# payakorn/InteriorPointMethod

Hardware: AMD Instinct MI355X
Metric: IPM iterations/sec (m=4096,n=8192 dense LP) (higher is better)
Workload: dtype f64; 1 GPU; dense synthetic LP m=4096 n=8192 fp64, seed 0, start x=s=1 y=0 (BASELINE.json configs[1]); replicas per GPU

## Files before the change

interiorpointmethod_amd/csrc/ff_schedule.h:

```cpp
#pragma once
#include <stdint.h>
#include <stdio.h>
#include <stdlib.h>

#include <math.h>

#include <algorithm>
#include <limits>
#include <queue>
#include <set>
#include <string>
#include <vector>

namespace ipm {

struct FFItem {
    unsigned char type;
    unsigned char i, c;
    unsigned char q;
    union {
        struct { unsigned char j0, j1, flags, seq; } t;
        struct { unsigned short s0, s1; } f;
    };
};
enum { FF_F = 0, FF_T = 1, FF_D = 2 };
enum { FF_INIT = 1, FF_ADD_BASE = 2, FF_PANEL = 4, FF_SIG_DIAG = 8 };
constexpr int FF_MAX_NBLK = 96;

#if defined(__HIPCC__)
#define FF_HD __host__ __device__
#else
#define FF_HD
#endif
FF_HD inline int ff_tile(int i, int c) { return i * (i + 1) / 2 + c; }

struct FFWords {
    static constexpr unsigned ticket = 0;
    static constexpr unsigned role = 3;
    static constexpr unsigned maxbits = 8;
    static constexpr unsigned dcount = 10;
    static constexpr unsigned dbg = 24;
    static constexpr unsigned dbg_end = 32;
    static constexpr unsigned fcount = 32;
    size_t tprog;
    size_t lfinal;
    size_t dready;
    size_t potrfdone;
    size_t count;
    FF_HD explicit FFWords(int nblk) {
        const size_t ntile = (size_t)nblk * ((size_t)nblk + 1) / 2;
        tprog = fcount + ntile; lfinal = tprog + ntile; dready = lfinal + (size_t)nblk; potrfdone = dready + (size_t)nblk;
        count = potrfdone + (size_t)nblk;
    }
    FF_HD static const unsigned* base_of_dbg(const unsigned* dbg_words) { return dbg_words - dbg; }
};

struct FFModel {
    double f_over = 6.1, f_stage = 4.02;
    double f_stage_half = 2.1;
    double t_over = 7.0, t_col = 15.9;
    double t_rmw = 1.0, t_panel = 18.3;
    double t_base = 2.3;
    double d_item = 130.0;
    double gap = 0.8, handoff = 1.0;
    double potrf = 36.8, cpanel = 7.3, cupdate = 7.3;
    int batch = 4;
    int tail = 2;
    double stagger = 0.3;
    int nstages = 512;
    int q_last = 0;
};

struct FFSchedule {
    std::vector<FFItem> items;
    std::vector<int> tile_items;
    std::vector<int> tile_q;
    double makespan_us = 0.0;
    double form_end_us = 0.0;
};

inline int ff_limit(int i, int c) { return (i == c) ? (c > 0 ? c - 1 : 0) : c; }
inline bool ff_needs_panel(int i, int c) { return i > c + 1; }

inline void ff_build_schedule(int nblk, int Q, int W, const FFModel& M_in, FFSchedule& out, int Qmax = 0) {
    if (Qmax < Q) Qmax = Q;
    const double INF = std::numeric_limits<double>::infinity();
    const int ntile = nblk * (nblk + 1) / 2;
    FFModel Mx = M_in;
    if (const char* e = getenv("IPM_FF_BATCH")) Mx.batch = std::max(1, atoi(e));
    if (const char* e = getenv("IPM_FF_TAIL")) Mx.tail = std::max(1, atoi(e));
    if (const char* e = getenv("IPM_FF_STAGGER")) Mx.stagger = std::min(0.9, std::max(0.0, atof(e)));
    if (const char* e = getenv("IPM_FF_Q_LAST")) Mx.q_last = std::max(0, atoi(e));
    if (const char* e = getenv("IPM_FF_MODEL")) {
        std::string spec(e);
        size_t p0 = 0;
        while (p0 < spec.size()) {
            size_t p1 = spec.find(',', p0); if (p1 == std::string::npos) p1 = spec.size();
            const std::string kv = spec.substr(p0, p1 - p0);
            const size_t eq = kv.find('=');
            if (eq != std::string::npos) {
                const std::string k = kv.substr(0, eq); const double v = atof(kv.c_str() + eq + 1);
                struct { const char* n; double* p; } tab[] = {{"f_over", &Mx.f_over}, {"f_stage", &Mx.f_stage}, {"f_stage_half", &Mx.f_stage_half}, {"t_over", &Mx.t_over}, {"t_col", &Mx.t_col},
                    {"t_rmw", &Mx.t_rmw}, {"t_panel", &Mx.t_panel}, {"t_base", &Mx.t_base}, {"d_item", &Mx.d_item}, {"potrf", &Mx.potrf},
                    {"cpanel", &Mx.cpanel}, {"cupdate", &Mx.cupdate}, {"handoff", &Mx.handoff}, {"gap", &Mx.gap}};
                for (auto& t : tab) if (k == t.n) *t.p = v;
            }
            p0 = p1 + 1;
        }
    }
    const FFModel& M = Mx;
    enum Kind { K_F, K_T, K_D, K_POTRF, K_CPANEL, K_CUPDATE };
    struct Node {
        Kind kind; int i = 0, c = 0, q = 0, j0 = 0, j1 = 0, flags = 0, seq = 0, s0 = 0, s1 = 0;
        double dur = 0.0, bl = 0.0, est = 0.0, fin = 0.0;
        int npred = 0, left = 0;
        std::vector<int> succ;
    };
    std::vector<Node> nd;
    nd.reserve((size_t)ntile * 6 + 4 * (size_t)nblk);
    auto add = [&](Kind k, double dur) { Node x; x.kind = k; x.dur = dur; x.fin = INF; nd.push_back(x); return (int)nd.size() - 1; };
    auto edge = [&](int a, int b) { nd[(size_t)a].succ.push_back(b); nd[(size_t)b].npred++; };
    std::vector<int> potrf((size_t)nblk), cpan, cupd;
    for (int k = 0; k < nblk; ++k) { potrf[(size_t)k] = add(K_POTRF, M.potrf + M.handoff); nd.back().i = k; }
    cpan.resize((size_t)nblk - 1); cupd.resize((size_t)nblk - 1);
    for (int k = 0; k + 1 < nblk; ++k) { cpan[(size_t)k] = add(K_CPANEL, M.cpanel + M.handoff); nd.back().i = k; }
    for (int k = 0; k + 1 < nblk; ++k) { cupd[(size_t)k] = add(K_CUPDATE, M.cupdate + M.handoff); nd.back().i = k; }
    for (int k = 0; k + 1 < nblk; ++k) { edge(potrf[(size_t)k], cpan[(size_t)k]); edge(cpan[(size_t)k], cupd[(size_t)k]); edge(cupd[(size_t)k], potrf[(size_t)k + 1]); }
    std::vector<std::vector<int>> titems((size_t)ntile);
    std::vector<int> lprod((size_t)ntile, -1);
    for (int i = 0; i < nblk; ++i)
        for (int c = 0; c <= i; ++c) {
            const int lim = ff_limit(i, c);
            const bool pan = ff_needs_panel(i, c);
            std::vector<std::pair<int, int>> cuts;
            const int nb_end = std::max(0, lim - M.tail);
            int j = 0;
            while (j + M.batch <= nb_end) { cuts.emplace_back(j, j + M.batch); j += M.batch; }
            if (j < nb_end) { cuts.emplace_back(j, nb_end); j = nb_end; }
            while (j < lim) { cuts.emplace_back(j, j + 1); ++j; }
            if (cuts.empty()) cuts.emplace_back(0, 0);
            std::vector<int>& ids = titems[(size_t)ff_tile(i, c)];
            for (size_t s = 0; s < cuts.size(); ++s) {
                const bool last = s + 1 == cuts.size();
                const int id = add(K_T, M.t_over + M.t_col * (cuts[s].second - cuts[s].first) + (s ? M.t_rmw : 0.0) + ((last && pan) ? M.t_panel : 0.0) + M.handoff + M.gap);
                Node& x = nd[(size_t)id];
                x.i = i; x.c = c; x.j0 = cuts[s].first; x.j1 = cuts[s].second; x.seq = (int)s + 1;
                x.flags = (s == 0 ? FF_INIT : 0) | ((last && pan) ? FF_PANEL : 0) | ((last && i == 0 && c == 0) ? FF_SIG_DIAG : 0);
                if (s) edge(ids.back(), id);
                ids.push_back(id);
            }
            if (pan) lprod[(size_t)ff_tile(i, c)] = ids.back();
        }
    for (int k = 0; k + 1 < nblk; ++k) {
        lprod[(size_t)ff_tile(k + 1, k)] = cpan[(size_t)k];
        edge(titems[(size_t)ff_tile(k + 1, k)].back(), cpan[(size_t)k]);
        edge(titems[(size_t)ff_tile(k + 1, k + 1)].back(), cupd[(size_t)k]);
    }
    edge(titems[0].back(), potrf[0]);
    for (int t = 0; t < ntile; ++t)
        for (int id : titems[(size_t)t]) {
            const int i = nd[(size_t)id].i, c = nd[(size_t)id].c, j1 = nd[(size_t)id].j1;
            if (j1 > nd[(size_t)id].j0) {
                edge(lprod[(size_t)ff_tile(i, j1 - 1)], id);
                if (c != i) edge(lprod[(size_t)ff_tile(c, j1 - 1)], id);
            }
            if (nd[(size_t)id].flags & FF_PANEL) edge(potrf[(size_t)c], id);
        }
    std::vector<int> base_item((size_t)ntile);
    for (int t = 0; t < ntile; ++t) { const std::vector<int>& ids = titems[(size_t)t]; base_item[(size_t)t] = ids.size() == 1 ? ids[0] : ids[ids.size() - 2]; }
    std::vector<int> fch;
    out.tile_q.assign((size_t)ntile, 0);
    {
        int npairs = 0;
        for (int i = 0; i < nblk; i += 2)
            for (int c = 0; c <= std::min(i + 1, nblk - 1); ++c) {
                int q = (M.q_last > 0 && i + 2 >= nblk) ? M.q_last : Q;
                q = std::max(1, std::min(std::min(q, Qmax), M.nstages));
                const double phi = std::fmod(npairs * 0.381966, 1.0);
                ++npairs;
                std::vector<int> cut((size_t)q + 1, 0);
                double tot = 0.0, acc = 0.0;
                std::vector<double> len((size_t)q);
                for (int k = 0; k < q; ++k) { len[(size_t)k] = 1.0 + M.stagger * (2.0 * std::fmod((double)k / q + phi, 1.0) - 1.0); tot += len[(size_t)k]; }
                for (int k = 0; k < q; ++k) { acc += len[(size_t)k]; cut[(size_t)k + 1] = (int)(M.nstages * acc / tot + 0.5); }
                cut[(size_t)q] = M.nstages;
                for (int k = 0; k < q; ++k) {
                    const bool half = c > i || i + 1 >= nblk;
                    const int id = add(K_F, M.f_over + (half ? M.f_stage_half : M.f_stage) * (cut[(size_t)k + 1] - cut[(size_t)k]) + M.gap);
                    Node& x = nd[(size_t)id];
                    x.i = i; x.c = c; x.q = k; x.s0 = cut[(size_t)k]; x.s1 = cut[(size_t)k + 1];
                    fch.push_back(id);
                    for (int r = i; r <= i + 1; ++r)
                        if (r >= c && r < nblk) { edge(id, base_item[(size_t)ff_tile(r, c)]); out.tile_q[(size_t)ff_tile(r, c)]++; }
                }
            }
    }
    for (int t = 0; t < ntile; ++t) { Node& x = nd[(size_t)base_item[(size_t)t]]; x.flags |= FF_ADD_BASE; x.dur += M.t_base * out.tile_q[(size_t)t]; }
    std::vector<int> ditems;
    for (int i = 0; i < nblk; ++i) { const int id = add(K_D, M.d_item + M.gap); nd[(size_t)id].i = i; edge(id, potrf[0]); ditems.push_back(id); }
    const int N = (int)nd.size();
    {
        std::vector<int> order, indeg((size_t)N), stack;
        order.reserve((size_t)N);
        for (int u = 0; u < N; ++u) { indeg[(size_t)u] = nd[(size_t)u].npred; if (!indeg[(size_t)u]) stack.push_back(u); }
        while (!stack.empty()) {
            const int u = stack.back(); stack.pop_back(); order.push_back(u);
            for (int v : nd[(size_t)u].succ) if (--indeg[(size_t)v] == 0) stack.push_back(v);
        }
        if ((int)order.size() != N) { out.items.clear(); return; }
        for (size_t k = order.size(); k-- > 0;) {
            Node& x = nd[(size_t)order[k]];
            double b = 0.0;
            for (int v : x.succ) b = std::max(b, nd[(size_t)v].bl);
            x.bl = x.dur + b;
        }
    }
    typedef std::pair<double, int> PI;
    std::priority_queue<PI, std::vector<PI>, std::greater<PI>> avail_F;
    std::set<PI> avail_T;
    for (int id : fch) avail_F.push(PI(-nd[(size_t)id].bl, id));
    for (int u = 0; u < N; ++u) nd[(size_t)u].left = nd[(size_t)u].npred;
    std::vector<int> rel;
    auto release = [&](int u0) {
        rel.clear(); rel.push_back(u0);
        while (!rel.empty()) {
            const int u = rel.back(); rel.pop_back();
            for (int v : nd[(size_t)u].succ) {
                Node& y = nd[(size_t)v];
                y.est = std::max(y.est, nd[(size_t)u].fin);
                if (--y.left == 0) {
                    if (y.kind == K_T) avail_T.insert(PI(-y.bl, v));
                    else if (y.kind != K_F && y.kind != K_D) {
                        y.fin = y.est + y.dur;
                        rel.push_back(v);
                    }
                }
            }
        }
    };
    for (int t = 0; t < ntile; ++t) { const int id = titems[(size_t)t][0]; if (nd[(size_t)id].left == 0) avail_T.insert(PI(-nd[(size_t)id].bl, id)); }
    typedef std::pair<double, int> Ev;
    std::priority_queue<Ev, std::vector<Ev>, std::greater<Ev>> free_at;
    for (int w = 0; w < W; ++w) free_at.push(Ev(0.0, w));
    out.items.clear();
    size_t nT = 0, doneT = 0, nextD = 0;
    for (int t = 0; t < ntile; ++t) nT += titems[(size_t)t].size();
    std::vector<int> order_out;
    int guard = 0;
    while (doneT < nT || !avail_F.empty() || nextD < ditems.size()) {
        const Ev ev = free_at.top(); free_at.pop();
        const double t = ev.first;
        if (nextD < ditems.size()) {
            const int v = ditems[nextD++];
            nd[(size_t)v].fin = t + nd[(size_t)v].dur;
            order_out.push_back(v); release(v);
            free_at.push(Ev(nd[(size_t)v].fin, ev.second));
            continue;
        }
        int pick = -1;
        for (const PI& p : avail_T) if (nd[(size_t)p.second].est <= t) { pick = p.second; break; }
        if (pick >= 0 && !avail_F.empty() && -avail_F.top().first > nd[(size_t)pick].bl) pick = -1;
        if (pick < 0 && !avail_F.empty()) {
            const int v = avail_F.top().second; avail_F.pop();
            nd[(size_t)v].fin = t + nd[(size_t)v].dur;
            out.form_end_us = std::max(out.form_end_us, nd[(size_t)v].fin);
            order_out.push_back(v); release(v);
            free_at.push(Ev(nd[(size_t)v].fin, ev.second));
            continue;
        }
        if (pick < 0) {
            if (avail_T.empty()) {
                if (++guard > 64 * W * nblk) break;
                free_at.push(Ev(t + 5.0, ev.second));
                continue;
            }
            double best = INF;
            for (const PI& p : avail_T) if (nd[(size_t)p.second].est < best) { best = nd[(size_t)p.second].est; pick = p.second; }
        }
        Node& x = nd[(size_t)pick];
        avail_T.erase(PI(-x.bl, pick));
        x.fin = std::max(t, x.est) + x.dur;
        order_out.push_back(pick); ++doneT;
        release(pick);
        free_at.push(Ev(x.fin, ev.second));
    }
    out.tile_items.assign((size_t)ntile, 0);
    for (int t = 0; t < ntile; ++t) out.tile_items[(size_t)t] = (int)titems[(size_t)t].size();
    out.makespan_us = 0.0;
    for (int v : order_out) {
        const Node& x = nd[(size_t)v];
        FFItem it{};
        it.i = (unsigned char)x.i; it.c = (unsigned char)x.c;
        if (x.kind == K_F) { it.type = FF_F; it.q = (unsigned char)x.q; it.f.s0 = (unsigned short)x.s0; it.f.s1 = (unsigned short)x.s1; }
        else if (x.kind == K_D) { it.type = FF_D; }
        else { it.type = FF_T; it.t.j0 = (unsigned char)x.j0; it.t.j1 = (unsigned char)x.j1; it.t.flags = (unsigned char)x.flags; it.t.seq = (unsigned char)x.seq; }
        out.items.push_back(it);
    }
    for (int k = 0; k < nblk; ++k) out.makespan_us = std::max(out.makespan_us, nd[(size_t)potrf[(size_t)k]].fin);
}

}
```

interiorpointmethod_amd/csrc/form_factor.h:

```cpp
#pragma once
#include <hip/hip_runtime.h>
#include <stdint.h>

#include "ff_schedule.h"
#include "gemm_nt_f64.h"
#include "handoff.h"
#include "potrf_f64.h"

namespace ipm {

constexpr int FF_THREADS = 512;
constexpr int FF_BK = 32, FF_LDT = FF_BK + 2;
constexpr int FF_OP = 128 * FF_LDT;
constexpr int FF_LDS_DOUBLES = 4 * FF_OP;

struct FFArgs {
    const double* A; int64_t lda;
    const double* d;
    double* B; int64_t ldb;
    const double* invD;
    double* slab;
    const FFItem* items; int nitems;
    unsigned* ticket;
    unsigned* fcount;
    unsigned* tprog;
    unsigned* lfinal;
    unsigned* dready;
    const unsigned* potrfdone;
    unsigned* timeout;
    unsigned* dbg;
    unsigned dbg_words;
    long long* prof;
    long long* trace;
    const int* done;
    int nblk, Q, nstages;
    int m;
    const int* tile_q;
    unsigned long long* maxbits;
    unsigned* dcount;
};

__device__ __forceinline__ void ff_wait_ge(const unsigned* p, unsigned v, unsigned* timeout, unsigned* dbg = nullptr, unsigned item = 0,
                                           unsigned kind = 0, unsigned nw = 0) {
    (void)handoff_wait<2, false>([=] { return handoff_load(p) >= v; }, {timeout, dbg}, [=] {
        handoff_record_ge(dbg, item, kind, v, p);
        const unsigned* live = FFWords::base_of_dbg(dbg);
        unsigned* snap = const_cast<unsigned*>(live) + nw;
        for (unsigned w = 0; w < nw; ++w) snap[w] = handoff_load(live + w);
    });
}

constexpr int FF_BASE_DEPTH = 4;

template <bool SCALE, bool SRC_REGS>
__device__ __forceinline__ void ff_gemm(const double* __restrict__ Pg, int64_t ldp, const double* __restrict__ Qg, int64_t ldq,
                                        const double* __restrict__ w, int ns, double* lds, f64x4 (&acc)[4][2],
                                        const f64x4 (*src)[2]) {
    const int tid = threadIdx.x, lane = tid & 63;
    const int wave = __builtin_amdgcn_readfirstlane(tid >> 6);
    const int wm = wave >> 2, wn = wave & 3;
    const int fr = lane & 15, fk = lane >> 4;
    double* Ps = lds;
    double* Qs = lds + 2 * FF_OP;
    const int ch = tid & 15, r0 = tid >> 4;
    const double* pP = SRC_REGS ? nullptr : Pg + (int64_t)r0 * ldp + ch * 2;
    const double* pQ = Qg + (int64_t)r0 * ldq + ch * 2;
    f64x2 pr[4], qr[4], wr;
    auto load_stage = [&](int s) {
        if (SCALE) wr = *reinterpret_cast<const f64x2*>(w + (int64_t)s * FF_BK + ch * 2);
#pragma unroll
        for (int u = 0; u < 4; ++u) qr[u] = *reinterpret_cast<const f64x2*>(pQ + (int64_t)u * 32 * ldq + (int64_t)s * FF_BK);
        if (!SRC_REGS) {
#pragma unroll
            for (int u = 0; u < 4; ++u) pr[u] = *reinterpret_cast<const f64x2*>(pP + (int64_t)u * 32 * ldp + (int64_t)s * FF_BK);
        }
    };
    auto store_stage = [&](int s, int buf) {
#pragma unroll
        for (int u = 0; u < 4; ++u) {
            f64x2 v = qr[u];
            if (SCALE) { v.x *= wr.x; v.y *= wr.y; }
            *reinterpret_cast<f64x2*>(Qs + buf * FF_OP + (r0 + 32 * u) * FF_LDT + ch * 2) = v;
        }
        if (!SRC_REGS) {
#pragma unroll
            for (int u = 0; u < 4; ++u) *reinterpret_cast<f64x2*>(Ps + buf * FF_OP + (r0 + 32 * u) * FF_LDT + ch * 2) = pr[u];
        } else if (wn == s) {
#pragma unroll
            for (int i = 0; i < 4; ++i)
#pragma unroll
                for (int j = 0; j < 2; ++j)
#pragma unroll
                    for (int q = 0; q < 4; ++q)
                        Ps[buf * FF_OP + (wm * 64 + i * 16 + fk + 4 * q) * FF_LDT + j * 16 + fr] = src[i][j][q];
        }
    };
    load_stage(0);
    store_stage(0, 0);
    __syncthreads();
    for (int s = 0; s < ns; ++s) {
        const int buf = s & 1;
        if (s + 1 < ns) load_stage(s + 1);
        const double* pa = Ps + buf * FF_OP + (wm * 64 + fr) * FF_LDT + fk;
        const double* qb = Qs + buf * FF_OP + (wn * 32 + fr) * FF_LDT + fk;
#pragma unroll
        for (int kk = 0; kk < FF_BK / 4; ++kk) {
            double a[4], b[2];
#pragma unroll
            for (int i = 0; i < 4; ++i) a[i] = pa[i * 16 * FF_LDT + kk * 4];
#pragma unroll
            for (int j = 0; j < 2; ++j) b[j] = qb[j * 16 * FF_LDT + kk * 4];
#pragma unroll
            for (int i = 0; i < 4; ++i)
#pragma unroll
                for (int j = 0; j < 2; ++j) acc[i][j] = __builtin_amdgcn_mfma_f64_16x16x4f64(a[i], b[j], acc[i][j], 0, 0, 0);
        }
        if (s + 1 < ns) store_stage(s + 1, buf ^ 1);
        __syncthreads();
    }
}

template <bool SCALE, bool HEAD>
__device__ __forceinline__ void ff_gemm_pipe(const double* __restrict__ Pg, int64_t ldp, const double* __restrict__ Qg, int64_t ldq,
                                             const double* __restrict__ w, int ns, double* lds, f64x4 (&acc)[4][2]) {
    const int tid = threadIdx.x, lane = tid & 63;
    const int wave = __builtin_amdgcn_readfirstlane(tid >> 6);
    const int wm = wave >> 2, wn = wave & 3;
    const int fr = lane & 15, fk = lane >> 4;
    double* Ps = lds;
    double* Qs = lds + 2 * FF_OP;
    const int ch = tid & 15, r0 = tid >> 4;
    const double* pP = Pg + (int64_t)r0 * ldp + ch * 2;
    const double* pQ = Qg + (int64_t)r0 * ldq + ch * 2;
    f64x2 pr[4], qr[4], wr;
    auto issue_loads = [&](int s) {
        if (SCALE) wr = *reinterpret_cast<const f64x2*>(w + (int64_t)s * FF_BK + ch * 2);
#pragma unroll
        for (int u = 0; u < 4; ++u) qr[u] = *reinterpret_cast<const f64x2*>(pQ + (int64_t)u * 32 * ldq + (int64_t)s * FF_BK);
#pragma unroll
        for (int u = 0; u < 4; ++u) pr[u] = *reinterpret_cast<const f64x2*>(pP + (int64_t)u * 32 * ldp + (int64_t)s * FF_BK);
    };
    const int st_off = r0 * FF_LDT + ch * 2;
    auto store_q = [&](int buf, int u) {
        f64x2 v = qr[u];
        if (SCALE) { v.x *= wr.x; v.y *= wr.y; }
        *reinterpret_cast<f64x2*>(Qs + buf * FF_OP + u * 32 * FF_LDT + st_off) = v;
    };
    auto store_p = [&](int buf, int u) { *reinterpret_cast<f64x2*>(Ps + buf * FF_OP + u * 32 * FF_LDT + st_off) = pr[u]; };
    const int fa_off = (wm * 64 + fr) * FF_LDT + fk, fb_off = (wn * 32 + fr) * FF_LDT + fk;
    double fa[2][4], fb[2][2];
    auto read_frags = [&](int set, int buf, int kk) {
        const double* pa = Ps + buf * FF_OP + fa_off + kk * 4;
        const double* qb = Qs + buf * FF_OP + fb_off + kk * 4;
#pragma unroll
        for (int i = 0; i < 4; ++i) fa[set][i] = pa[i * 16 * FF_LDT];
#pragma unroll
        for (int j = 0; j < 2; ++j) fb[set][j] = qb[j * 16 * FF_LDT];
    };
    auto mfma8 = [&](int set) {
#pragma unroll
        for (int i = 0; i < 4; ++i)
#pragma unroll
            for (int j = 0; j < 2; ++j) acc[i][j] = __builtin_amdgcn_mfma_f64_16x16x4f64(fa[set][i], fb[set][j], acc[i][j], 0, 0, 0);
    };
    auto mfma_row = [&](int set, int i) {
#pragma unroll
        for (int j = 0; j < 2; ++j) acc[i][j] = __builtin_amdgcn_mfma_f64_16x16x4f64(fa[set][i], fb[set][j], acc[i][j], 0, 0, 0);
    };
    issue_loads(0);
#pragma unroll
    for (int u = 0; u < 4; ++u) { store_q(0, u); store_p(0, u); }
    __syncthreads();
    if (HEAD) issue_loads(min(1, ns - 1));
    else if (1 < ns) issue_loads(1);
    read_frags(0, 0, 0);
    for (int s = 0; s < ns; ++s) {
        const int buf = s & 1;
        const bool more = HEAD || s + 1 < ns;
#pragma unroll
        for (int kk = 0; kk < 6; ++kk) {
            read_frags((kk + 1) & 1, buf, kk + 1);
            __builtin_amdgcn_sched_barrier(0);
            mfma8(kk & 1);
            __builtin_amdgcn_sched_barrier(0);
        }
        read_frags(1, buf, 7);
        __builtin_amdgcn_sched_barrier(0);
#pragma unroll
        for (int i = 0; i < 4; ++i) {
#pragma unroll
            for (int j = 0; j < 2; ++j) acc[i][j] = __builtin_amdgcn_mfma_f64_16x16x4f64(fa[0][i], fb[0][j], acc[i][j], 0, 0, 0);
            if (more) { store_q(buf ^ 1, i); store_p(buf ^ 1, i); }
            __builtin_amdgcn_sched_barrier(0);
        }
        __syncthreads();
        if constexpr (HEAD) {
            mfma_row(1, 0);
            __builtin_amdgcn_sched_barrier(0);
            issue_loads(min(s + 2, ns - 1));
            __builtin_amdgcn_sched_barrier(0);
            mfma_row(1, 1);
            __builtin_amdgcn_sched_barrier(0);
            read_frags(0, buf ^ 1, 0);
            __builtin_amdgcn_sched_barrier(0);
            mfma_row(1, 2);
            mfma_row(1, 3);
            __builtin_amdgcn_sched_barrier(0);
        } else {
            if (s + 2 < ns) issue_loads(s + 2);
            if (more) read_frags(0, buf ^ 1, 0);
            __builtin_amdgcn_sched_barrier(0);
            mfma8(1);
            __builtin_amdgcn_sched_barrier(0);
        }
    }
    __syncthreads();
}

constexpr int FF_PBK = 16, FF_PLDT = FF_PBK + 2;
constexpr int FF_POP_P = 256 * FF_PLDT, FF_POP_Q = 128 * FF_PLDT;
static_assert(2 * (FF_POP_P + FF_POP_Q) <= FF_LDS_DOUBLES, "pair engine LDS");

template <bool HEAD, bool HALF = false>
__device__ __forceinline__ void ff_gemm_pair(const double* __restrict__ P0, const double* __restrict__ P1, const double* __restrict__ Qg,
                                             int64_t ld, const double* __restrict__ w, int ns, double* lds, f64x4 (&acc)[4][4], int lh = 0) {
    static_assert(HEAD || !HALF, "the half-live engine exists on the MFMA-first schedule only");
    constexpr int NP = HALF ? 2 : 4;
    const int tid = threadIdx.x, lane = tid & 63;
    const int wave = __builtin_amdgcn_readfirstlane(tid >> 6);
    const int wm = wave >> 1, wn = wave & 1;
    const int fr = lane & 15, fk = lane >> 4;
    double* Ps = lds;
    double* Qs = lds + 2 * FF_POP_P;
    const int ch = tid & 7, r0 = tid >> 3;
    const double* pP0 = P0 + (int64_t)r0 * ld + ch * 2;
    const double* pP1 = HALF ? nullptr : P1 + (int64_t)r0 * ld + ch * 2;
    const double* pQ = Qg + (int64_t)r0 * ld + ch * 2;
    f64x2 pr[NP], qr[2], wr;
    auto issue_loads = [&](int s) {
        wr = *reinterpret_cast<const f64x2*>(w + (int64_t)s * FF_PBK + ch * 2);
#pragma unroll
        for (int u = 0; u < 2; ++u) qr[u] = *reinterpret_cast<const f64x2*>(pQ + (int64_t)u * 64 * ld + (int64_t)s * FF_PBK);
#pragma unroll
        for (int u = 0; u < 2; ++u) pr[u] = *reinterpret_cast<const f64x2*>(pP0 + (int64_t)u * 64 * ld + (int64_t)s * FF_PBK);
        if constexpr (!HALF) {
#pragma unroll
            for (int u = 0; u < 2; ++u) pr[2 + u] = *reinterpret_cast<const f64x2*>(pP1 + (int64_t)u * 64 * ld + (int64_t)s * FF_PBK);
        }
    };
    const int st_off = r0 * FF_PLDT + ch * 2;
    auto store_q = [&](int buf, int u) {
        f64x2 v = qr[u];
        v.x *= wr.x; v.y *= wr.y;
        *reinterpret_cast<f64x2*>(Qs + buf * FF_POP_Q + u * 64 * FF_PLDT + st_off) = v;
    };
    const int st_off_p = HALF ? st_off + lh * 128 * FF_PLDT : st_off;
    auto store_p = [&](int buf, int u) { *reinterpret_cast<f64x2*>(Ps + buf * FF_POP_P + u * 64 * FF_PLDT + st_off_p) = pr[u]; };
    const int fa_off = (wm * 64 + fr) * FF_PLDT + fk, fb_off = (wn * 64 + fr) * FF_PLDT + fk;
    double fa[2][4], fb[2][4];
    auto read_frags = [&](int set, int buf, int kk) {
        const double* pa = Ps + buf * FF_POP_P + fa_off + kk * 4;
        const double* qb = Qs + buf * FF_POP_Q + fb_off + kk * 4;
#pragma unroll
        for (int i = 0; i < 4; ++i) fa[set][i] = pa[i * 16 * FF_PLDT];
#pragma unroll
        for (int j = 0; j < 4; ++j) fb[set][j] = qb[j * 16 * FF_PLDT];
    };
    auto mfma16 = [&](int set) {
#pragma unroll
        for (int i = 0; i < 4; ++i)
#pragma unroll
            for (int j = 0; j < 4; ++j) acc[i][j] = __builtin_amdgcn_mfma_f64_16x16x4f64(fa[set][i], fb[set][j], acc[i][j], 0, 0, 0);
    };
    auto mfma_row = [&](int set, int i) {
#pragma unroll
        for (int j = 0; j < 4; ++j) acc[i][j] = __builtin_amdgcn_mfma_f64_16x16x4f64(fa[set][i], fb[set][j], acc[i][j], 0, 0, 0);
    };
    issue_loads(0);
#pragma unroll
    for (int u = 0; u < 2; ++u) store_q(0, u);
#pragma unroll
    for (int u = 0; u < NP; ++u) store_p(0, u);
    __syncthreads();
    if (HEAD) issue_loads(min(1, ns - 1));
    else if (1 < ns) issue_loads(1);
    if (HALF && (wm >> 1) != lh) {
        for (int s = 0; s < ns; ++s) {
            const int buf = s & 1;
#pragma unroll
            for (int u = 0; u < 2; ++u) { store_q(buf ^ 1, u); store_p(buf ^ 1, u); }
            __syncthreads();
            issue_loads(min(s + 2, ns - 1));
        }
        __syncthreads();
        return;
    }
    read_frags(0, 0, 0);
    for (int s = 0; s < ns; ++s) {
        const int buf = s & 1;
        const bool more = HEAD || s + 1 < ns;
        read_frags(1, buf, 1);
        __builtin_amdgcn_sched_barrier(0);
        mfma16(0);
        __builtin_amdgcn_sched_barrier(0);
        read_frags(0, buf, 2);
        __builtin_amdgcn_sched_barrier(0);
        mfma16(1);
        __builtin_amdgcn_sched_barrier(0);
        read_frags(1, buf, 3);
        __builtin_amdgcn_sched_barrier(0);
#pragma unroll
        for (int i = 0; i < 4; ++i) {
#pragma unroll
            for (int j = 0; j < 4; ++j) acc[i][j] = __builtin_amdgcn_mfma_f64_16x16x4f64(fa[0][i], fb[0][j], acc[i][j], 0, 0, 0);
            if (more) { if (i < 2) store_q(buf ^ 1, i); if (i < NP) store_p(buf ^ 1, i); }
            __builtin_amdgcn_sched_barrier(0);
        }
        __syncthreads();
        if constexpr (HEAD) {
            mfma_row(1, 0);
            __builtin_amdgcn_sched_barrier(0);
            issue_loads(min(s + 2, ns - 1));
            __builtin_amdgcn_sched_barrier(0);
            mfma_row(1, 1);
            __builtin_amdgcn_sched_barrier(0);
            read_frags(0, buf ^ 1, 0);
            __builtin_amdgcn_sched_barrier(0);
            mfma_row(1, 2);
            mfma_row(1, 3);
            __builtin_amdgcn_sched_barrier(0);
        } else {
            if (s + 2 < ns) issue_loads(s + 2);
            if (more) read_frags(0, buf ^ 1, 0);
            __builtin_amdgcn_sched_barrier(0);
            mfma16(1);
            __builtin_amdgcn_sched_barrier(0);
        }
    }
    __syncthreads();
}


struct FFChain {
    double* B; int64_t ldb; double* invD;
    const unsigned long long* maxbits; const unsigned* dcount; double* maxdiag_out;
    const unsigned* dready; unsigned* potrfdone;
    unsigned* timeout; unsigned* dbg; long long* trace;
    double eps, big, shift_rel;
    int* fixed; const int* done;
    int nblk, m;
};

__device__ __forceinline__ void ff_chain_role(const FFChain& c, double* lds) {
    static_assert(NB * WLD + NB + 2 <= FF_LDS_DOUBLES, "chain role LDS");
    double* W = lds;
    double* dinv_s = lds + NB * WLD;
    double* maxdiag_p = dinv_s + NB;
    const int tid = threadIdx.x;
    if (tid == 0) {
        ff_wait_ge(c.dcount, (unsigned)c.nblk, c.timeout, c.dbg, 9000u, HK_DCOUNT, 0);
        handoff_acquire();
        const double mx = __longlong_as_double((long long)__hip_atomic_load(c.maxbits, __ATOMIC_RELAXED, __HIP_MEMORY_SCOPE_AGENT));
        *maxdiag_p = mx;
        *c.maxdiag_out = mx;
    }
    __syncthreads();
    for (int k = 0; k < c.nblk; ++k) {
        PotrfDiag a;
        a.Bkk = c.B + (int64_t)k * NB * (c.ldb + 1); a.ld = c.ldb;
        a.inv = c.invD + (int64_t)k * NB * NB;
        a.maxdiag = maxdiag_p; a.eps = c.eps; a.big = c.big; a.shift_rel = c.shift_rel;
        a.fixed = c.fixed; a.done = nullptr; a.stamps = nullptr;
        a.wait_on = c.dready + k; a.wait_count = 4u; a.signal = c.potrfdone + k; a.timeout = c.timeout; a.dbg = c.dbg; a.dbg_tag = (unsigned)k;
        a.trace = c.trace ? c.trace + 12 * (size_t)k : nullptr;
        const int real = c.m - k * NB;
        a.nt = (c.shift_rel != 0.0 || real >= NB) ? NB / 16 : (real + 15) / 16 < 1 ? 1 : (real + 15) / 16;
        a.rows = real;
        potrf_diag_body<false>(a, W, dinv_s);
        __syncthreads();
    }
}

struct FFCrit {
    double* B; int64_t ldb; const double* invD;
    const unsigned* tprog; const int* tile_items;
    const unsigned* potrfdone; unsigned* lfinal; unsigned* dready;
    unsigned* timeout; unsigned* dbg; long long* trace;
    const int* done;
    int nblk;
};
constexpr int FF_CRIT_WGS = 4;

__device__ __forceinline__ void ff_crit_role(const FFCrit& c, const int strip, double* lds) {
    static_assert(2 * (32 + 128) * (32 + 2) <= FF_LDS_DOUBLES, "critical role LDS");
    const int tid = threadIdx.x;
    GemmNT g;
    g.w = nullptr; g.M = 128; g.N = 128; g.K = 128; g.lower = 0; g.unit_diag_from = -1; g.done = nullptr;
    g.n_direct = FF_CRIT_WGS; g.split_p = 1; g.chunk_stages = 128 / 32; g.slab = nullptr; g.tile_offset = 0; g.tile_order = nullptr;
    g.sP = g.sQ = g.sC = 0; g.batch = 1; g.sP2 = g.sQ2 = g.sC2 = 0; g.batch2 = 1;
    g.wait_on = nullptr; g.wait_count = 0; g.timeout = nullptr; g.dbg = nullptr; g.dbg_tag = 0; g.trace = nullptr;
    for (int k = 0; k + 1 < c.nblk; ++k) {
        double* panel = c.B + (int64_t)(k + 1) * 128 * c.ldb + (int64_t)k * 128;
        long long* tr = (c.trace && strip == 0 && tid == 0) ? c.trace + 12 * (size_t)k : nullptr;
        if (tr) tr[4] = (long long)wall_clock64();
        if (tid == 0) {
            const int t = ff_tile(k + 1, k);
            ff_wait_ge(c.tprog + t, (unsigned)c.tile_items[t], c.timeout, c.dbg, 1000u + (unsigned)k, HK_GEMM, 0);
            ff_wait_ge(c.potrfdone + k, 1u, c.timeout, c.dbg, 1000u + (unsigned)k, HK_GEMM, 0);
            handoff_acquire();
        }
        __syncthreads();
        if (tr) tr[5] = (long long)wall_clock64();
        g.P = panel; g.ldp = c.ldb; g.Q = c.invD + (int64_t)k * 128 * 128; g.ldq = 128;
        g.C = panel; g.ldc = c.ldb; g.alpha = 1.0; g.beta = 0.0; g.signal = c.lfinal + (k + 1);
        gemm_nt_body<32, 128, 32, 1, 8, false>(g, strip, 0, 0, lds);
        if (tr) { tr[6] = (long long)wall_clock64(); tr[8] = tr[6]; }
        if (tid == 0) {
            const int t = ff_tile(k + 1, k + 1);
            ff_wait_ge(c.lfinal + (k + 1), 4u * (unsigned)(k + 1), c.timeout, c.dbg, 2000u + (unsigned)k, HK_GEMM, 0);
            ff_wait_ge(c.tprog + t, (unsigned)c.tile_items[t], c.timeout, c.dbg, 2000u + (unsigned)k, HK_GEMM, 0);
            handoff_acquire();
        }
        __syncthreads();
        if (tr) tr[9] = (long long)wall_clock64();
        g.P = panel; g.ldp = c.ldb; g.Q = panel; g.ldq = c.ldb;
        g.C = c.B + (int64_t)(k + 1) * 128 * (c.ldb + 1); g.ldc = c.ldb; g.alpha = -1.0; g.beta = 1.0; g.signal = c.dready + (k + 1);
        gemm_nt_body<32, 128, 32, 1, 8, false>(g, strip, 0, 0, lds);
        if (tr) tr[10] = (long long)wall_clock64();
        __syncthreads();
    }
}

enum { FFP_TICKET = 0, FFP_FGEMM, FFP_FSTORE, FFP_TWAIT, FFP_TGEMM, FFP_TBASE, FFP_PWAIT, FFP_PGEMM, FFP_TSTORE, FFP_NF, FFP_NT, FFP_TOTAL };
#define FF_PROF(slot) do { if (TRACE && g.prof && tid == 0) { const long long t_ = __builtin_amdgcn_s_memtime(); g.prof[(size_t)blockIdx.x * 16 + (slot)] += t_ - tprev; tprev = t_; } } while (0)
#define FF_TRACE(slot) do { if (TRACE && g.trace && tid == 0) g.trace[(size_t)n * 4 + (slot)] = (long long)wall_clock64(); } while (0)

struct FFRoles { FFChain chain; FFCrit crit; unsigned* role; };

template <bool TRACE, bool HEAD>
__device__ __forceinline__ void form_factor_body(const FFArgs& g, const FFRoles& r) {
    __shared__ __attribute__((aligned(16))) double lds[FF_LDS_DOUBLES];
    __shared__ unsigned ticket_s;
    if (threadIdx.x == 0) ticket_s = __hip_atomic_fetch_add(r.role, 1u, __ATOMIC_RELAXED, __HIP_MEMORY_SCOPE_AGENT);
    __syncthreads();
    const unsigned role = ticket_s;
    __syncthreads();
    if (role == 0u) { ff_chain_role(r.chain, lds); return; }
    if (role <= (unsigned)FF_CRIT_WGS) { ff_crit_role(r.crit, (int)role - 1, lds); return; }
    const int tid = threadIdx.x, lane = tid & 63;
    const int wave = __builtin_amdgcn_readfirstlane(tid >> 6);
    const int wm = wave >> 2, wn = wave & 3;
    const int fr = lane & 15, fk = lane >> 4;
    const int er = wm * 64 + fk, ec = wn * 32 + fr;

    long long tprev = (TRACE && g.prof) ? __builtin_amdgcn_s_memtime() : 0;
    const long long tstart = tprev;
    for (;;) {
        constexpr unsigned SEL_EXIT = 0xffffffffu;
        if (tid == 0) {
            const unsigned n0 = __hip_atomic_fetch_add(g.ticket, 1u, __ATOMIC_RELAXED, __HIP_MEMORY_SCOPE_AGENT);
            ticket_s = n0 < (unsigned)g.nitems ? n0 : SEL_EXIT;
        }
        __syncthreads();
        const unsigned n = ticket_s;
        __syncthreads();
        if (n == SEL_EXIT) { if (TRACE && g.prof && tid == 0) g.prof[(size_t)blockIdx.x * 16 + FFP_TOTAL] = __builtin_amdgcn_s_memtime() - tstart; return; }
        const FFItem it = g.items[n];
        FF_PROF(FFP_TICKET);
        FF_TRACE(0);
        if (TRACE && g.trace && tid == 0) g.trace[(size_t)n * 4 + 3] = (long long)blockIdx.x;
        const int ti = it.i, tc = it.c;
        const int tile = ff_tile(ti, tc);
        if (it.type == FF_D) {
            double mx = 0.0;
            const int ncols = g.nstages * FF_PBK;
            for (int rr = wave; rr < 128; rr += 8) {
                const int row = ti * 128 + rr;
                if (row >= g.m) break;
                const double* a = g.A + (int64_t)row * g.lda;
                double s0 = 0.0, s1 = 0.0, s2 = 0.0, s3 = 0.0;
                int kq = lane * 2;
                for (; kq + 384 < ncols; kq += 512) {
                    const f64x2 a0 = *reinterpret_cast<const f64x2*>(a + kq), a1 = *reinterpret_cast<const f64x2*>(a + kq + 128);
                    const f64x2 a2 = *reinterpret_cast<const f64x2*>(a + kq + 256), a3 = *reinterpret_cast<const f64x2*>(a + kq + 384);
                    const f64x2 d0 = *reinterpret_cast<const f64x2*>(g.d + kq), d1 = *reinterpret_cast<const f64x2*>(g.d + kq + 128);
                    const f64x2 d2 = *reinterpret_cast<const f64x2*>(g.d + kq + 256), d3 = *reinterpret_cast<const f64x2*>(g.d + kq + 384);
                    s0 = __builtin_fma(a0.x * a0.x, d0.x, s0); s0 = __builtin_fma(a0.y * a0.y, d0.y, s0);
                    s1 = __builtin_fma(a1.x * a1.x, d1.x, s1); s1 = __builtin_fma(a1.y * a1.y, d1.y, s1);
                    s2 = __builtin_fma(a2.x * a2.x, d2.x, s2); s2 = __builtin_fma(a2.y * a2.y, d2.y, s2);
                    s3 = __builtin_fma(a3.x * a3.x, d3.x, s3); s3 = __builtin_fma(a3.y * a3.y, d3.y, s3);
                }
                for (; kq < ncols; kq += 128) {
                    const f64x2 va = *reinterpret_cast<const f64x2*>(a + kq);
                    const f64x2 vd = *reinterpret_cast<const f64x2*>(g.d + kq);
                    s0 = __builtin_fma(va.x * va.x, vd.x, s0);
                    s0 = __builtin_fma(va.y * va.y, vd.y, s0);
                }
                double sacc = (s0 + s1) + (s2 + s3);
#pragma unroll
                for (int o = 32; o > 0; o >>= 1) sacc += __shfl_xor(sacc, o, 64);
                mx = (sacc > mx) ? sacc : mx;
            }
            if (lane == 0) atomicMax(g.maxbits, (unsigned long long)__double_as_longlong(mx));
            handoff_publish_begin();
            if (tid == 0) __hip_atomic_fetch_add(g.dcount, 1u, __ATOMIC_RELAXED, __HIP_MEMORY_SCOPE_AGENT);
            FF_TRACE(2);
            continue;
        }
        if (it.type == FF_F) {
            const bool up = ti >= tc, lo = ti + 1 < g.nblk;
            const int s0 = it.f.s0, s1 = min(g.nstages, (int)it.f.s1);
            f64x4 pacc[4][4];
#pragma unroll
            for (int i = 0; i < 4; ++i)
#pragma unroll
                for (int j = 0; j < 4; ++j) pacc[i][j] = (f64x4){0.0, 0.0, 0.0, 0.0};
            const int r_up = up ? ti : ti + 1, r_lo = lo ? ti + 1 : ti;
            if (s1 > s0) {
                if (HEAD && !(up && lo))
                    ff_gemm_pair<HEAD, HEAD>(g.A + (int64_t)r_up * 128 * g.lda + (int64_t)s0 * FF_PBK, nullptr, g.A + (int64_t)tc * 128 * g.lda + (int64_t)s0 * FF_PBK,
                                             g.lda, g.d + (int64_t)s0 * FF_PBK, s1 - s0, lds, pacc, up ? 0 : 1);
                else
                    ff_gemm_pair<HEAD>(g.A + (int64_t)r_up * 128 * g.lda + (int64_t)s0 * FF_PBK, g.A + (int64_t)r_lo * 128 * g.lda + (int64_t)s0 * FF_PBK,
                                       g.A + (int64_t)tc * 128 * g.lda + (int64_t)s0 * FF_PBK, g.lda, g.d + (int64_t)s0 * FF_PBK, s1 - s0, lds, pacc);
            }
            FF_PROF(FFP_FGEMM);
            {
                const int pm = wave >> 1, pn = wave & 1;
                const int half = pm >> 1;
                if (half == 0 ? up : lo) {
                    const int tl = ff_tile(ti + half, tc);
                    double* sb = g.slab + ((size_t)tl * g.Q + it.q) * (128 * 128) + (size_t)((pm & 1) * 2 + pn) * 4096 + lane * 2;
#pragma unroll
                    for (int i = 0; i < 4; ++i)
#pragma unroll
                        for (int j = 0; j < 4; ++j)
#pragma unroll
                            for (int hq = 0; hq < 2; ++hq)
                                *reinterpret_cast<f64x2*>(sb + ((i * 4 + j) * 2 + hq) * 128) = (f64x2){pacc[i][j][2 * hq], pacc[i][j][2 * hq + 1]};
                }
            }
            handoff_publish_begin();
            if (tid == 0) {
                if (up) __hip_atomic_fetch_add(g.fcount + ff_tile(ti, tc), 1u, __ATOMIC_RELAXED, __HIP_MEMORY_SCOPE_AGENT);
                if (lo) __hip_atomic_fetch_add(g.fcount + ff_tile(ti + 1, tc), 1u, __ATOMIC_RELAXED, __HIP_MEMORY_SCOPE_AGENT);
                if (TRACE && g.prof) g.prof[(size_t)blockIdx.x * 16 + FFP_NF] += 1;
            }
            FF_PROF(FFP_FSTORE);
            FF_TRACE(2);
            continue;
        }

        f64x4 acc[4][2];
#pragma unroll
        for (int i = 0; i < 4; ++i)
#pragma unroll
            for (int j = 0; j < 2; ++j) acc[i][j] = (f64x4){0.0, 0.0, 0.0, 0.0};
        const int j0 = it.t.j0, j1 = it.t.j1;
        const int flags = it.t.flags, seq = it.t.seq;
        int qn_v = 0;
        if (HEAD && (flags & FF_ADD_BASE)) qn_v = g.tile_q[tile];
        if (tid == 0) {
            if (flags & FF_ADD_BASE) ff_wait_ge(g.fcount + tile, (unsigned)g.tile_q[tile], g.timeout, g.dbg, n, HK_FCOUNT, g.dbg_words);
            if (!(flags & FF_INIT)) ff_wait_ge(g.tprog + tile, (unsigned)seq - 1u, g.timeout, g.dbg, n, HK_TPROG, g.dbg_words);
            if (j1 > j0) {
                ff_wait_ge(g.lfinal + ti, 4u * (unsigned)j1, g.timeout, g.dbg, n, HK_LFINAL_ROW, g.dbg_words);
                if (tc != ti) ff_wait_ge(g.lfinal + tc, 4u * (unsigned)j1, g.timeout, g.dbg, n, HK_LFINAL_COL, g.dbg_words);
            }
            handoff_acquire();
        }
        __syncthreads();
        const int qn_s = __builtin_amdgcn_readfirstlane(qn_v);
        FF_PROF(FFP_TWAIT);
        FF_TRACE(1);
        if (j1 > j0)
            ff_gemm_pipe<false, HEAD>(g.B + (int64_t)ti * 128 * g.ldb + (int64_t)j0 * 128, g.ldb,
                                g.B + (int64_t)tc * 128 * g.ldb + (int64_t)j0 * 128, g.ldb, nullptr, (j1 - j0) * (128 / FF_BK), lds, acc);
        FF_PROF(FFP_TGEMM);
        double* bt = g.B + ((int64_t)ti * 128 + er) * g.ldb + (int64_t)tc * 128 + ec;
        f64x4 val[4][2];
#pragma unroll
        for (int i = 0; i < 4; ++i)
#pragma unroll
            for (int j = 0; j < 2; ++j) val[i][j] = (f64x4){0.0, 0.0, 0.0, 0.0};
        if (!(flags & FF_INIT)) {
#pragma unroll
            for (int i = 0; i < 4; ++i)
#pragma unroll
                for (int j = 0; j < 2; ++j)
#pragma unroll
                    for (int q = 0; q < 4; ++q) val[i][j][q] = bt[(int64_t)(i * 16 + 4 * q) * g.ldb + j * 16];
        }
        if constexpr (HEAD) {
            if (flags & FF_ADD_BASE) {
                constexpr int D = FF_BASE_DEPTH;
                static_assert(D == 1 || D == 2 || D == 4, "a ring slot serves the same register groups in every slab");
                const int qn = qn_s;
                unsigned loff = (unsigned)((wm * 2 + (wn >> 1)) * 4096 + (wn & 1) * 512 + lane * 2);
                asm volatile("" : "+v"(loff));
                const double* sb = g.slab + ((size_t)tile * g.Q * (128 * 128) + loff);
                f64x2 ring[D][4];
                auto fill = [&](const double* s, int i) {
#pragma unroll
                    for (int jh = 0; jh < 4; ++jh) ring[i % D][jh] = *reinterpret_cast<const f64x2*>(s + (i * 8 + jh) * 128);
                };
                auto add = [&](int i) {
#pragma unroll
                    for (int jh = 0; jh < 4; ++jh) { val[i][jh >> 1][2 * (jh & 1)] += ring[i % D][jh].x; val[i][jh >> 1][2 * (jh & 1) + 1] += ring[i % D][jh].y; }
                };
#pragma unroll
                for (int i = 0; i < D; ++i) fill(sb, i);
                for (int c = 0; c + 1 < qn; ++c, sb += 128 * 128) {
#pragma unroll
                    for (int i = 0; i < 4; ++i) { add(i); fill(sb + ((i + D) >> 2) * (128 * 128), (i + D) & 3); }
                }
#pragma unroll
                for (int i = 0; i < 4; ++i) { add(i); if (i + D < 4) fill(sb, i + D); }
            }
        } else if (flags & FF_ADD_BASE) {
            const int qn = g.tile_q[tile];
            for (int c = 0; c < qn; ++c) {
                const double* sb = g.slab + ((size_t)tile * g.Q + c) * (128 * 128) + (size_t)(wm * 2 + (wn >> 1)) * 4096 + lane * 2;
#pragma unroll
                for (int i = 0; i < 4; ++i)
#pragma unroll
                    for (int j = 0; j < 2; ++j)
#pragma unroll
                        for (int hq = 0; hq < 2; ++hq) {
                            const f64x2 v = *reinterpret_cast<const f64x2*>(sb + ((i * 4 + (wn & 1) * 2 + j) * 2 + hq) * 128);
                            val[i][j][2 * hq] += v.x; val[i][j][2 * hq + 1] += v.y;
                        }
            }
        }
#pragma unroll
        for (int i = 0; i < 4; ++i)
#pragma unroll
            for (int j = 0; j < 2; ++j) val[i][j] -= acc[i][j];
        if (ti == tc && (flags & FF_ADD_BASE)) {
#pragma unroll
            for (int i = 0; i < 4; ++i)
#pragma unroll
                for (int j = 0; j < 2; ++j)
#pragma unroll
                    for (int q = 0; q < 4; ++q) {
                        const int r = er + i * 16 + 4 * q, c = ec + j * 16;
                        if (r == c && ti * 128 + r >= g.m) val[i][j][q] = 1.0;
                    }
        }
        FF_PROF(FFP_TBASE);
        if (flags & FF_PANEL) {
            if (tid == 0) {
                ff_wait_ge(g.potrfdone + tc, 1u, g.timeout, g.dbg, n, HK_POTRFDONE, g.dbg_words);
                handoff_acquire();
            }
            __syncthreads();
            FF_PROF(FFP_PWAIT);
#pragma unroll
            for (int i = 0; i < 4; ++i)
#pragma unroll
                for (int j = 0; j < 2; ++j) acc[i][j] = (f64x4){0.0, 0.0, 0.0, 0.0};
            ff_gemm<false, true>(nullptr, 0, g.invD + (int64_t)tc * 128 * 128, 128, nullptr, 128 / FF_BK, lds, acc, val);
#pragma unroll
            for (int i = 0; i < 4; ++i)
#pragma unroll
                for (int j = 0; j < 2; ++j) val[i][j] = acc[i][j];
            FF_PROF(FFP_PGEMM);
        }
#pragma unroll
        for (int i = 0; i < 4; ++i)
#pragma unroll
            for (int j = 0; j < 2; ++j)
#pragma unroll
                for (int q = 0; q < 4; ++q) bt[(int64_t)(i * 16 + 4 * q) * g.ldb + j * 16] = val[i][j][q];
        handoff_publish_begin();
        if (tid == 0) {
            __hip_atomic_store(g.tprog + tile, (unsigned)seq, __ATOMIC_RELAXED, __HIP_MEMORY_SCOPE_AGENT);
            if (flags & FF_PANEL) __hip_atomic_fetch_add(g.lfinal + ti, 4u, __ATOMIC_RELAXED, __HIP_MEMORY_SCOPE_AGENT);
            if (flags & FF_SIG_DIAG) __hip_atomic_fetch_add(g.dready + ti, 10u, __ATOMIC_RELAXED, __HIP_MEMORY_SCOPE_AGENT);
            if (TRACE && g.prof) g.prof[(size_t)blockIdx.x * 16 + FFP_NT] += 1;
        }
        FF_PROF(FFP_TSTORE);
        FF_TRACE(2);
    }
}

template <bool TRACE>
__global__ __launch_bounds__(FF_THREADS, 2) void form_factor_roles_kernel(FFArgs g, FFRoles r) {
    if (g.done && *g.done) return;
    form_factor_body<TRACE, false>(g, r);
}
template <bool TRACE>
__global__ __launch_bounds__(FF_THREADS, 2) void form_factor_roles_kernel_mfma_first(FFArgs g, FFRoles r) {
    if (g.done && *g.done) return;
    form_factor_body<TRACE, true>(g, r);
}

__global__ __launch_bounds__(64) void ff_gate_kernel(const unsigned* flag, unsigned value, unsigned* timeout, const int* done) {
    if (done && *done) return;
    if (threadIdx.x == 0) {
        ff_wait_ge(flag, value, timeout);
        handoff_acquire<false>();
    }
}

}
```

Measured before the change: 277.9 iterations/s.

## Use triangular-aware GEMM for panel solve against inverse diagonal block

Adds a specialized panel GEMM that multiplies the tile by the triangular inverse diagonal block and skips MFMA work on the known-zero half. It also reorganizes the wave-to-output mapping so each wave owns a 16-row strip across all 8 column blocks, and writes results directly to B. The scheduler's panel cost estimate is lowered to match. It adds per-stage register staging of source values into LDS and trace instrumentation, and relies on the inverse block being strictly triangular in the assumed orientation.

```diff
diff --git a/interiorpointmethod_amd/csrc/ff_schedule.h b/interiorpointmethod_amd/csrc/ff_schedule.h
--- a/interiorpointmethod_amd/csrc/ff_schedule.h
+++ b/interiorpointmethod_amd/csrc/ff_schedule.h
@@ -59,7 +59,7 @@
     double f_over = 6.1, f_stage = 4.02;
     double f_stage_half = 2.1;
     double t_over = 7.0, t_col = 15.9;
-    double t_rmw = 1.0, t_panel = 18.3;
+    double t_rmw = 1.0, t_panel = 11.8;
     double t_base = 2.3;
     double d_item = 130.0;
     double gap = 0.8, handoff = 1.0;
diff --git a/interiorpointmethod_amd/csrc/form_factor.h b/interiorpointmethod_amd/csrc/form_factor.h
--- a/interiorpointmethod_amd/csrc/form_factor.h
+++ b/interiorpointmethod_amd/csrc/form_factor.h
@@ -52,6 +52,8 @@
 
 constexpr int FF_BASE_DEPTH = 4;
 
+constexpr bool FF_TRI_PANEL = true;
+
 template <bool SCALE, bool SRC_REGS>
 __device__ __forceinline__ void ff_gemm(const double* __restrict__ Pg, int64_t ldp, const double* __restrict__ Qg, int64_t ldq,
                                         const double* __restrict__ w, int ns, double* lds, f64x4 (&acc)[4][2],
@@ -116,6 +118,60 @@
                 for (int j = 0; j < 2; ++j) acc[i][j] = __builtin_amdgcn_mfma_f64_16x16x4f64(a[i], b[j], acc[i][j], 0, 0, 0);
         }
         if (s + 1 < ns) store_stage(s + 1, buf ^ 1);
+        __syncthreads();
+    }
+}
+
+__device__ __forceinline__ void ff_gemm_tri(const double* __restrict__ Qg, double* lds, f64x4 (&acc)[8], const f64x4 (*src)[2]) {
+    constexpr int NS = 128 / FF_BK;
+    const int tid = threadIdx.x, lane = tid & 63;
+    const int wave = __builtin_amdgcn_readfirstlane(tid >> 6);
+    const int wm = wave >> 2, wn = wave & 3;
+    const int fr = lane & 15, fk = lane >> 4;
+    double* Ps = lds;
+    double* Qs = lds + 2 * FF_OP;
+    unsigned ot = threadIdx.x;
+    asm volatile("" : "+v"(ot));
+    const int ch = ot & 15, r0 = ot >> 4;
+    const double* pQ = Qg + r0 * 128 + ch * 2;
+    f64x2 qr[4];
+    auto load_stage = [&](int s) {
+#pragma unroll
+        for (int u = 0; u < 4; ++u) qr[u] = *reinterpret_cast<const f64x2*>(pQ + u * 32 * 128 + s * FF_BK);
+    };
+    auto store_stage = [&](int s, int buf) {
+#pragma unroll
+        for (int u = 0; u < 4; ++u) *reinterpret_cast<f64x2*>(Qs + buf * FF_OP + (r0 + 32 * u) * FF_LDT + ch * 2) = qr[u];
+        if (wn == s) {
+#pragma unroll
+            for (int i = 0; i < 4; ++i)
+#pragma unroll
+                for (int j = 0; j < 2; ++j)
+#pragma unroll
+                    for (int q = 0; q < 4; ++q)
+                        Ps[buf * FF_OP + (wm * 64 + i * 16 + fk + 4 * q) * FF_LDT + j * 16 + fr] = src[i][j][q];
+        }
+    };
+    load_stage(0);
+    store_stage(0, 0);
+    __syncthreads();
+#pragma unroll
+    for (int s = 0; s < NS; ++s) {
+        const int buf = s & 1;
+        if (s + 1 < NS) load_stage(s + 1);
+        const double* pa = Ps + buf * FF_OP + (wave * 16 + fr) * FF_LDT + fk;
+        const double* qb = Qs + buf * FF_OP + fr * FF_LDT + fk;
+#pragma unroll
+        for (int kk = 0; kk < FF_BK / 4; ++kk) {
+            const int b0 = 2 * s + (kk >= 4 ? 1 : 0);
+            const double a = pa[kk * 4];
+            double b[8];
+#pragma unroll
+            for (int bb = b0; bb < 8; ++bb) b[bb] = qb[bb * 16 * FF_LDT + kk * 4];
+#pragma unroll
+            for (int bb = b0; bb < 8; ++bb) acc[bb] = __builtin_amdgcn_mfma_f64_16x16x4f64(a, b[bb], acc[bb], 0, 0, 0);
+        }
+        if (s + 1 < NS) store_stage(s + 1, buf ^ 1);
         __syncthreads();
     }
 }
@@ -509,6 +565,8 @@
         }
         if (it.type == FF_F) {
             const bool up = ti >= tc, lo = ti + 1 < g.nblk;
+            long long fcyc = 0;
+            if (TRACE && HEAD && g.trace && tid == 0) fcyc = __builtin_amdgcn_s_memtime();
             const int s0 = it.f.s0, s1 = min(g.nstages, (int)it.f.s1);
             f64x4 pacc[4][4];
 #pragma unroll
@@ -547,6 +605,7 @@
                 if (TRACE && g.prof) g.prof[(size_t)blockIdx.x * 16 + FFP_NF] += 1;
             }
             FF_PROF(FFP_FSTORE);
+            if (TRACE && HEAD && g.trace && tid == 0) g.trace[(size_t)n * 4 + 1] = __builtin_amdgcn_s_memtime() - fcyc;
             FF_TRACE(2);
             continue;
         }
@@ -648,6 +707,7 @@
                     }
         }
         FF_PROF(FFP_TBASE);
+        constexpr bool TRI = HEAD && FF_TRI_PANEL;
         if (flags & FF_PANEL) {
             if (tid == 0) {
                 ff_wait_ge(g.potrfdone + tc, 1u, g.timeout, g.dbg, n, HK_POTRFDONE, g.dbg_words);
@@ -655,23 +715,38 @@
             }
             __syncthreads();
             FF_PROF(FFP_PWAIT);
+            if constexpr (TRI) {
+                f64x4 pac[8];
+#pragma unroll
+                for (int b = 0; b < 8; ++b) pac[b] = (f64x4){0.0, 0.0, 0.0, 0.0};
+                ff_gemm_tri(g.invD + (int64_t)tc * 128 * 128, lds, pac, val);
+                FF_PROF(FFP_PGEMM);
+                double* bp = g.B + ((int64_t)ti * 128 + wave * 16 + fk) * g.ldb + (int64_t)tc * 128 + fr;
+#pragma unroll
+                for (int b = 0; b < 8; ++b)
+#pragma unroll
+                    for (int q = 0; q < 4; ++q) bp[(int64_t)(4 * q) * g.ldb + b * 16] = pac[b][q];
+            } else {
+#pragma unroll
+                for (int i = 0; i < 4; ++i)
+#pragma unroll
+                    for (int j = 0; j < 2; ++j) acc[i][j] = (f64x4){0.0, 0.0, 0.0, 0.0};
+                ff_gemm<false, true>(nullptr, 0, g.invD + (int64_t)tc * 128 * 128, 128, nullptr, 128 / FF_BK, lds, acc, val);
+#pragma unroll
+                for (int i = 0; i < 4; ++i)
+#pragma unroll
+                    for (int j = 0; j < 2; ++j) val[i][j] = acc[i][j];
+                FF_PROF(FFP_PGEMM);
+            }
+        }
+        if (!(TRI && (flags & FF_PANEL))) {
 #pragma unroll
             for (int i = 0; i < 4; ++i)
 #pragma unroll
-                for (int j = 0; j < 2; ++j) acc[i][j] = (f64x4){0.0, 0.0, 0.0, 0.0};
-            ff_gemm<false, true>(nullptr, 0, g.invD + (int64_t)tc * 128 * 128, 128, nullptr, 128 / FF_BK, lds, acc, val);
-#pragma unroll
-            for (int i = 0; i < 4; ++i)
-#pragma unroll
-                for (int j = 0; j < 2; ++j) val[i][j] = acc[i][j];
-            FF_PROF(FFP_PGEMM);
-        }
-#pragma unroll
-        for (int i = 0; i < 4; ++i)
-#pragma unroll
-            for (int j = 0; j < 2; ++j)
-#pragma unroll
-                for (int q = 0; q < 4; ++q) bt[(int64_t)(i * 16 + 4 * q) * g.ldb + j * 16] = val[i][j][q];
+                for (int j = 0; j < 2; ++j)
+#pragma unroll
+                    for (int q = 0; q < 4; ++q) bt[(int64_t)(i * 16 + 4 * q) * g.ldb + j * 16] = val[i][j][q];
+        }
         handoff_publish_begin();
         if (tid == 0) {
             __hip_atomic_store(g.tprog + tile, (unsigned)seq, __ATOMIC_RELAXED, __HIP_MEMORY_SCOPE_AGENT);
```

Measured after the change: 278.3 iterations/s (median of 4 runs). About the same (+0.1%).
